# codeandkey/kami

Hardware: AMD Instinct MI355X
Metric: NN leaf-evals/sec at batch 512 (119×8×8 planes), 1/2/4/8 MI355X (higher is better)
Workload: dtype bf16

## Files before the change

### kami_amd/csrc/kh_internal.h

```cpp
#pragma once
#include <hip/hip_runtime.h>
#include <stddef.h>
#include <stdint.h>

#include "../../include/kami_hip.h"

namespace kh {

void launch_encode_f32(const kh_board* d_boards, int n, float* d_planes, hipStream_t s);

void launch_gather_legal(const float* policy, const int32_t* offsets, const int32_t* actions,
                         float* priors, int B, hipStream_t s, const float* vfull = nullptr, int vstride = 0,
                         float* values = nullptr, const int* flags_in = nullptr, int* flags_out = nullptr);

void launch_signal(unsigned* host_word, unsigned serial, hipStream_t s);

struct SimpleLayer {
    const float* wt;
    const float* scale;
    const float* shift;
    int Ci, Co, taps;
    int relu;
};
void launch_simple_conv(const SimpleLayer& L, const float* in, const float* skip, float* out,
                        int B, hipStream_t s);
void launch_softmax4672(const float* logits, float* policy, int B, int* flags, hipStream_t s);
void launch_value_fc(const float* v64, const float* fcw, const float* fcb, float* value_full,
                     int B, int* flags, hipStream_t s);

constexpr int TW_NB = 2;
constexpr int TW_CP = 64;

struct TowerArgs {
    const float* in;
    const kh_board* boards;
    int B, F, R;
    const char* wstream;
    int nchunks;
    const float* params;
    int npar;
    const float* fcw4;
    const float* fcb;
    float* policy;
    float* vfull;
    float* logits;
    int* flags;
// ... 60 lines not shown
```

### kami_amd/csrc/tower8_mfma.hip

```cpp
#include "tower_common.h"

#include <atomic>

namespace kh {

using f32x4_t = float __attribute__((ext_vector_type(4)));
__device__ __forceinline__ void store_wt(f32x4_t* p, f32x4_t v) { asm volatile("global_store_dwordx4 %0, %1, off sc1" ::"v"(p), "v"(v) : "memory"); }
__device__ __forceinline__ void store_wt(float* p, float v) { asm volatile("global_store_dword %0, %1, off sc1" ::"v"(p), "v"(v) : "memory"); }

constexpr int T8_LAG = 1;
struct CPipe { unsigned ring; int cslot; };

__device__ __forceinline__ unsigned cpipe_advance(CPipe& p)
{
    p.cslot = (p.cslot + 1 == RING_D) ? 0 : p.cslot + 1;
    return p.ring + p.cslot * CHUNK;
}

__device__ __forceinline__ unsigned cpipe_step(CPipe& p)
{
    asm volatile("s_barrier" ::: "memory");
    __builtin_amdgcn_sched_barrier(0);
    p.cslot = (p.cslot + 1 == RING_D) ? 0 : p.cslot + 1;
    return p.ring + p.cslot * CHUNK;
// ... 8 lines not shown
    asm volatile("s_mov_b32 %0, m0\n\ts_mov_b32 m0, %3\n\ts_nop 0\n\t"
                 "global_load_lds_dwordx4 %1, %2\n\tglobal_load_lds_dwordx4 %1, %2 offset:1024\n\t"
                 "global_load_lds_dwordx4 %1, %2 offset:2048\n\tglobal_load_lds_dwordx4 %1, %2 offset:3072\n\t"
                 "s_mov_b32 m0, %0"
                 : "=&s"(keep) : "v"(voff), "s"(sbase), "s"(dst) : "memory");
    p.next = (p.next + 1 == p.nch) ? 0 : p.next + 1;
    p.islot = (p.islot + 1 == RING_D) ? 0 : p.islot + 1;
}

template <int VMX>
__device__ __forceinline__ void hpipe_step(Pipe& p, int hw, int lane)
{
    asm volatile("s_waitcnt vmcnt(%0)" ::"n"(4 * (RING_D - 3 - T8_LAG) + VMX) : "memory");
    asm volatile("s_barrier" ::: "memory");
    pipe_issue4(p, hw, lane);
}

template <typename T, int TAPS, int KS, int MS, int PAR, int NREG = 0, bool CF = false, int TAILV = 0>
__device__ __forceinline__ void gemm8_layer(CPipe& p, const char* smem, int lane, unsigned b_base, int stride,
                                            f32x16 (&acc)[MS], typename Elem<T>::vec8 (&A)[2][8],
                                            const typename Elem<T>::vec8* breg = nullptr)
{
    using V = typename Elem<T>::vec8;
    using S = LayerShape<TAPS, KS, MS>;
    constexpr int KPC = S::KPC;
    constexpr int NF = KPC * MS;
    V B[2][KPC];
#pragma unroll
    for (int k = 0; k < KPC; ++k) {
        if (k < NREG) B[PAR][k] = breg[k];
        else B[PAR][k] = *reinterpret_cast<const V*>(smem + b_base + b_offset<TAPS, KS, CF>(k, stride));
    }
#pragma unroll
    for (int n = 0; n < S::NCH; ++n) {
        const int cur = (PAR + n) & 1, nxt = cur ^ 1;
        const unsigned a_off = cpipe_step(p) + lane * 16;
#pragma unroll
        for (int f = 0; f < 8; ++f)
            if (n + 1 == S::NCH || f < NF) A[nxt][f] = *reinterpret_cast<const V*>(smem + a_off + f * 1024);
        if (n + 1 < S::NCH) {
#pragma unroll
            for (int k = 0; k < KPC; ++k) {
                if ((n + 1) * KPC + k < NREG) B[nxt][k] = breg[(n + 1) * KPC + k];
                else B[nxt][k] = *reinterpret_cast<const V*>(smem + b_base + b_offset<TAPS, KS, CF>((n + 1) * KPC + k, stride));
            }
        }
        if (TAILV > 0 && n == S::NCH - 1) {
#pragma unroll
            for (int ms = 0; ms < MS; ++ms)
#pragma unroll
                for (int k = 0; k < KPC; ++k) acc[ms] = Elem<T>::mfma(A[cur][k * MS + ms], B[cur][k], acc[ms]);
#pragma unroll
            for (int i = 0; i < KPC; ++i) {
                __builtin_amdgcn_sched_group_barrier(0x100, 2, 0);
                __builtin_amdgcn_sched_group_barrier(0x008, 1, 0);
            }
#pragma unroll
            for (int i = 0; i < (MS - 1) * KPC; ++i) {
                __builtin_amdgcn_sched_group_barrier(0x008, 1, 0);
                if (i > 0) __builtin_amdgcn_sched_group_barrier(0x002, TAILV, 0);
            }
            continue;
        }
#pragma unroll
        for (int k = 0; k < KPC; ++k)
#pragma unroll
            for (int ms = 0; ms < MS; ++ms) acc[ms] = Elem<T>::mfma(A[cur][k * MS + ms], B[cur][k], acc[ms]);
#pragma unroll
        for (int i = 0; i < NF; ++i) {
            __builtin_amdgcn_sched_group_barrier(0x100, 2, 0);
            __builtin_amdgcn_sched_group_barrier(0x008, 1, 0);
        }
    }
}

template <typename T, int PAR>
__device__ __forceinline__ void gemm8_dummy(CPipe& p, const char* smem, int lane, typename Elem<T>::vec8 (&A)[2][8])
{
    using V = typename Elem<T>::vec8;
    const unsigned a_off = cpipe_step(p) + lane * 16;
#pragma unroll
    for (int f = 0; f < 8; ++f) A[PAR ^ 1][f] = *reinterpret_cast<const V*>(smem + a_off + f * 1024);
}


enum { BM_RASTER = 0, BM_CENTRE = 1, BM_QUARTERS = 2 };
template <int TAPS, int KS, int BM>
__device__ __forceinline__ constexpr unsigned b_off8(int kk, int stride)
// ... 166 lines not shown
    constexpr int cur = CURP, nxt = CURP ^ 1;
    const unsigned a_off = cpipe_step(p) + lane * 16;
    T8_RDA(nxt, 0, a_off); T8_RDA(nxt, 1, a_off); acc[0] = Elem<T>::mfma(A[cur][0], B[cur][0], acc[0]); T8_FENCE();
    T8_RDA(nxt, 2, a_off); T8_RDA(nxt, 3, a_off); acc[0] = Elem<T>::mfma(A[cur][2], B[cur][1], acc[0]); T8_FENCE();
    T8_RDA(nxt, 4, a_off); T8_RDA(nxt, 5, a_off); acc[0] = Elem<T>::mfma(A[cur][4], B[cur][2], acc[0]); T8_FENCE();
    T8_RDA(nxt, 6, a_off); T8_RDA(nxt, 7, a_off); acc[0] = Elem<T>::mfma(A[cur][6], B[cur][3], acc[0]); T8_FENCE();
    acc[1] = Elem<T>::mfma(A[cur][1], B[cur][0], acc[1]); T8_FENCE();
    acc[1] = Elem<T>::mfma(A[cur][3], B[cur][1], acc[1]); T8_FENCE();
    xk.o[0][0] = epi_group<T, EPI, 0>(acc[0], xf[0]); xk.o[0][1] = epi_group<T, EPI, 1>(acc[0], xf[0]);
    acc[1] = Elem<T>::mfma(A[cur][5], B[cur][2], acc[1]); T8_FENCE();
    xk.o[0][2] = epi_group<T, EPI, 2>(acc[0], xf[0]); xk.o[0][3] = epi_group<T, EPI, 3>(acc[0], xf[0]);
    acc[1] = Elem<T>::mfma(A[cur][7], B[cur][3], acc[1]); T8_FENCE();
    xk.o[1][0] = epi_group<T, EPI, 0>(acc[1], xf[1]); xk.o[1][1] = epi_group<T, EPI, 1>(acc[1], xf[1]);
    xk.o[1][2] = epi_group<T, EPI, 2>(acc[1], xf[1]); xk.o[1][3] = epi_group<T, EPI, 3>(acc[1], xf[1]);
}
#undef T8_RDA

template <int STRIDE>
__device__ __forceinline__ void zero_halo(char* base, int board_bytes, int t)
{
    const u32x4 z = { 0, 0, 0, 0 };
    for (int i = t; i < TW_NB * NPIX; i += 256) {
        const int pp = i % NPIX, yy = pp / PITCH, xx = pp % PITCH;
        if (yy >= 1 && yy <= 8 && xx >= 1 && xx <= 8) continue;
        char* d = base + (i / NPIX) * board_bytes + pp * STRIDE;
#pragma unroll
        for (int k = 0; k < STRIDE / 16; ++k) *reinterpret_cast<u32x4*>(d + k * 16) = z;
    }
}

// ... 41 lines not shown

template <typename T, int KS_STEM, bool LEGAL = false>
__global__ __launch_bounds__(512) void tower8_kernel(TowerArgs a)
{
    extern __shared__ __attribute__((aligned(16))) char smem[];
    constexpr int FP = KS_STEM * 16;
    constexpr int SSTR = FP * 2 + 16;
    constexpr int SBOARD = NPIX * SSTR;
    constexpr int ST_SIZE = st_size(FP);
    constexpr int LDS_PAR = LDS_ST + ST_SIZE;
    constexpr int LDS_L = LDS_X;
    using V = typename Elem<T>::vec8;
    constexpr int NSTEM = LayerShape<9, KS_STEM, 2>::NCH;
    constexpr int P1 = NSTEM & 1;
    constexpr int NLAYER = LayerShape<9, TW_CP / 16, 2>::NCH;
    constexpr int NPOL = LayerShape<1, TW_CP / 16, 4>::NCH + LayerShape<1, KH_POLICY_MID / 16, 3>::NCH + (P1 ? 1 : 0);

    const int tid = threadIdx.x;
    const int lane = tid & 63;
    const int wave = __builtin_amdgcn_readfirstlane(tid >> 6);
    const int ct = tid & 255;
    const int cw = wave & 3;
    const int R = a.R, F = a.F;

    float* par = reinterpret_cast<float*>(smem + LDS_PAR);
    const float* shift3 = par;
    const float* pshift1 = par + (1 + 2 * R) * TW_CP;
    const float* pbias2 = pshift1 + KH_POLICY_MID;
    const float* vw = pbias2 + 128;
    const float* vsh = vw + TW_CP;
    float* v64 = const_cast<float*>(vsh) + 4;
    float* red = v64 + TW_NB * 64;
    const int ngroups = (a.B + TW_NB - 1) / TW_NB;

    if (wave >= 6) {
        const int pt = tid & 127;
        for (int grp = blockIdx.x; grp < ngroups; grp += gridDim.x) {
            const int b0 = grp * TW_NB;
            if (KS_STEM == 8) {
                float4_u pl[4][8];
                const int lc = pt & 7;
                const int nb = min(TW_NB, a.B - b0);
                const char* gbase = reinterpret_cast<const char*>(a.in + (size_t)b0 * 64 * F);
                unsigned voff[8];
#pragma unroll
                for (int j = 0; j < 8; ++j) {
                    const int ip = (pt >> 3) + 16 * j;
                    voff[j] = (unsigned)((min(ip >> 6, nb - 1) * 64 + (ip & 63)) * F) * 4u;
                }
                const unsigned sdst = LDS_ST + ((((pt >> 6) + 1) * PITCH + ((pt >> 3) & 7) + 1) * SSTR) + 8 * lc;
                unsigned badmax = 0u;
// ... 92 lines not shown
                        for (int k = 0; k < 4; ++k) {
                            const float lo = vin[j][2 * k], hi = vin[j][2 * k + 1];
                            bad = bad || !__builtin_isfinite(lo) || !__builtin_isfinite(hi);
                            w[k] = pack2<T>(lo, hi);
                        }
                        o.x = w[0]; o.y = w[1]; o.z = w[2]; o.w = w[3];
                        *reinterpret_cast<u32x4*>(smem + LDS_ST + bb * SBOARD + (((p >> 3) + 1) * PITCH + (p & 7) + 1) * SSTR + (pt % CH) * 16) = o;
                    }
                    if (__any(bad) && lane == 0) raise_flag<LEGAL>(a, 0);
                }
                lds_barrier();
                for (int i = 0; i < NSTEM; ++i) asm volatile("s_barrier" ::: "memory");
            }
            const int nsteps = 2 * R * NLAYER + NPOL;
            for (int i = 0; i < nsteps; ++i) {
                asm volatile("s_barrier" ::: "memory");
                if (i == 0 && R > 0) {
                    for (int z = 0; z < 2; ++z) zero_halo<XSTR>(smem + LDS_ST, XBOARD, pt + 128 * z);
                    asm volatile("s_waitcnt lgkmcnt(0)" ::: "memory");
                }
            }
            helper_value_fc<LEGAL>(a, v64, b0, tid & 255, lane);
            asm volatile("s_barrier" ::: "memory");
        }
    } else if (wave >= 4) {
        const int hw = wave - 4;
        const int nsteps = NSTEM + 2 * R * NLAYER + NPOL;
        Pipe pipe;
        pipe.stream = a.wstream; pipe.nch = a.nchunks; pipe.next = 0; pipe.islot = 0; pipe.ring = LDS_RING;
#pragma unroll
        for (int i = 0; i < RING_D - 1; ++i) pipe_issue4(pipe, hw, lane);

        for (int grp = blockIdx.x; grp < ngroups; grp += gridDim.x) {
            asm volatile("s_waitcnt vmcnt(%0)\n\ts_barrier" ::"n"(4 * (RING_D - 3)) : "memory");
            for (int i = 0; i < nsteps; ++i) hpipe_step<0>(pipe, hw, lane);
// ... 55 lines not shown
                constexpr int BMS = KS_STEM == 8 ? BM_QUARTERS : BM_RASTER;
#pragma unroll
                for (int k = 0; k < 4; ++k) B[0][k] = *reinterpret_cast<const V*>(smem + sin + b_off8<9, KS_STEM, BMS>(k, SSTR));
                gemm8_steps<T, 9, KS_STEM, 2, 0, 0, BMS, 0, NSTEM - 1>(pipe, smem, lane, sin, SSTR, accA, A, B);
            }
            constexpr int CP1 = P1 ^ 1;
            for (int r = 0; r < R; ++r) {
                boundary<T, EPI_RESID, CP1>(pipe, smem, lane, accA, accB, sh0 + (1 + 2 * r) * TW_CP * 4, A, B, xf, xout_h, xin);
                gemm8_steps<T, 9, TW_CP / 16, 2, P1, 4, BM_CENTRE, 1, 8, true>(pipe, smem, lane, xin, XSTR, accB, A, B);
                boundary<T, EPI_PACK, P1>(pipe, smem, lane, accB, accA, sh0 + (2 + 2 * r) * TW_CP * 4, A, B, xf, tout_h, tin);
                gemm8_steps<T, 9, TW_CP / 16, 2, P1 ^ 1, 4, BM_CENTRE, 1, 8, true>(pipe, smem, lane, tin, XSTR, accA, A, B);
            }
            tower_tail<T, EPI_RESID, CP1>(pipe, smem, lane, accA, A, B, xf, xk);

            {
                f32x2 s01 = { 0.0f, 0.0f }, s23 = { 0.0f, 0.0f };
#pragma unroll
                for (int ms = 0; ms < 2; ++ms)
#pragma unroll
                    for (int g = 0; g < 4; ++g) {
                        using f32x4 = float __attribute__((ext_vector_type(4)));
                        const f32x4 w = *reinterpret_cast<const f32x4*>(vw + ms * 32 + 8 * g + 4 * h);
                        const f32x2 x01 = { xf[ms][4 * g + 0], xf[ms][4 * g + 1] }, x23 = { xf[ms][4 * g + 2], xf[ms][4 * g + 3] };
                        s01 = x01 * w.xy + s01;
                        s23 = x23 * w.zw + s23;
                    }
                const float part = (s01.x + s01.y) + (s23.x + s23.y);
                const unsigned pu = __float_as_uint(part);
                if ((pu & 0x7f800000u) == 0x7f800000u) raise_flag<LEGAL>(a, 0);
                const auto sw = __builtin_amdgcn_permlane32_swap(pu, pu, false, false);
                const float sv = __uint_as_float(sw[0]) + __uint_as_float(sw[1]);
                if (h == 0) v64[wb * 64 + py * 8 + px] = relu_nan(sv + vsh[0]);
            }

            Packed<4> pk;
            {
                f32x16 acc[4];
                V bf[4];
                packed_fragments<T, 2>(xk, bf);
                acc_init<4>(acc, pshift1, h);
                asm volatile("s_waitcnt lgkmcnt(0)" ::: "memory");
                gemm8_layer<T, 1, TW_CP / 16, 4, P1, 4>(pipe, smem, lane, 0, 0, acc, A, bf);
                epilogue_pack<T, 4>(acc, pk);
            }
            {
                f32x16 acc[3];
                V bf[8];
                packed_fragments<T, 4>(pk, bf);
                acc_init<3>(acc, pbias2, h);
                gemm8_layer<T, 1, KH_POLICY_MID / 16, 3, P1, 8>(pipe, smem, lane, 0, 0, acc, A, bf);
                if (P1) gemm8_dummy<T, 1>(pipe, smem, lane, A);
                float* lrow = reinterpret_cast<float*>(smem + LDS_L + wb * LBOARD) + (py * 8 + px) * KH_POLICY_PLANES;
                float m = -INFINITY;
#pragma unroll
                for (int ms = 0; ms < 3; ++ms)
#pragma unroll
                    for (int g = 0; g < 4; ++g)
#pragma unroll
                        for (int i = 0; i < 4; ++i) {
                            const int plane = ms * 32 + 8 * g + 4 * h + i;
                            if (plane < KH_POLICY_PLANES) {
                                lrow[plane] = acc[ms][4 * g + i];
                                m = fmaxf(m, acc[ms][4 * g + i]);
                            }
                        }
                m = wave_max_f(m);
                if (lane == 0) red[cw] = m;
                lds_barrier();
            }

            {
                const int bb = ct >> 7, tt = ct & 127;
                const bool live = (b0 + bb) < a.B;
                const float4* L4 = reinterpret_cast<const float4*>(smem + LDS_L + bb * LBOARD);
                constexpr int NQ = KH_PSIZE / 4;
                float4 v[10];
#pragma unroll
                for (int k = 0; k < 10; ++k) {
                    const int q = tt + 128 * k;
                    v[k] = (q < NQ) ? L4[q] : make_float4(-INFINITY, -INFINITY, -INFINITY, -INFINITY);
// ... 86 lines not shown
```

### kami_amd/csrc/weights.hip

```cpp
#include "engine.h"
#include "blob_layout.h"
#include "weights_pack.h"

#include <algorithm>
#include <atomic>
#include <cmath>
#include <cstring>
#include <thread>

namespace kh {
namespace {

struct ConvBN { const float *w, *b, *g, *be, *rm, *rv; };
struct HostNet {
    ConvBN stem;
    std::vector<ConvBN> res;
    ConvBN pconv;
    const float *p2w, *p2b;
    ConvBN vconv;
    const float *fcw, *fcb;
};

HostNet parse_blob(const float* blob, int F, int C, int R)
{
// ... 12 lines not shown
    n.fcw = take();
    n.fcb = take();
    return n;
}

void fold_bn(const ConvBN& c, int co, float* scale, float* shift)
{
    for (int i = 0; i < co; ++i) {
        const float s = c.g[i] / sqrtf(c.rv[i] + 1e-5f);
        scale[i] = s;
        shift[i] = (c.b[i] - c.rm[i]) * s + c.be[i];
    }
}

void pack_layer(std::vector<uint16_t>& out, int dtype, const float* w, const float* scale, int Co, int Ci,
                int taps, int KS, int MS, int ci0 = 0, bool centre_first = false, int perm = 0)
{
    int kstep = 0;
    for (int ti = 0; ti < taps; ++ti) {
        const int tap = !centre_first ? ti : (ti == 0 ? 4 : (ti <= 4 ? ti - 1 : ti));
        for (int ks = 0; ks < KS; ++ks, ++kstep)
            for (int ms = 0; ms < MS; ++ms)
                for (int l = 0; l < 64; ++l) {
                    const int r = l & 31, h = l >> 5;
                    for (int j = 0; j < 8; ++j) {
                        const int co = ms * 32 + r;
                        const int ci = ci0 + (kstep < perm ? 32 * (ks >> 1) + 8 * (2 * (ks & 1) + (j >> 2)) + 4 * h + (j & 3)
                                                           : ks * 16 + 8 * h + j);
                        float v = 0.0f;
                        if (co < Co && ci < Ci) v = w[((size_t)co * Ci + ci) * taps + tap] * (scale ? scale[co] : 1.0f);
                        out.push_back(dtype == KH_BF16 ? f2bf16(v) : f2f16(v));
                    }
                }
    }
}

void pack_layer_generic(uint16_t* o, int dtype, const float* w, const float* scale,
                        int Co, int Ci, int taps, int CoP, int CiP)
{
    const bool bf = dtype == KH_BF16;
    for (int cb = 0; cb < CoP / 64; ++cb)
        for (int slice = 0; slice < CiP / 64; ++slice)
            for (int tap = 0; tap < taps; ++tap)
                for (int kk = 0; kk < 4; ++kk)
                    for (int ms = 0; ms < 2; ++ms)
                        for (int l = 0; l < 64; ++l) {
                            const int r = l & 31, h = l >> 5, ks = slice * 4 + kk;
                            const int co = cb * 64 + ms * 32 + r, ci0 = ks * 16 + 8 * h;
// ... 45 lines not shown

enum Buf { B_TW_STREAM, B_TW_PAR, B_TW_FC4, B_LY_W, B_LY_W4, B_LY_W2B, B_LY_WH, B_LY_SHIFT, B_LY_MISC, B_SIMPLE, NBUF };

DevMem& buf_of(Weights& W, int b)
{
    DevMem* m[NBUF] = { &W.tw_stream, &W.tw_par, &W.tw_fc4, &W.ly_w, &W.ly_w4, &W.ly_w2b, &W.ly_wh, &W.ly_shift, &W.ly_misc, &W.simple };
    return *m[b];
}

struct FoldItem { ConvBN c; int co; };
struct FoldRef { int item = -1, shift = 0; };
struct PackItem {
    int buf; size_t off, bytes;
    int kind; const float* w; int fold;
    int Co, Ci, taps;
    int KS, MS, ci0, centre_first, perm, chunk_frags;
    int CoP, CiP, CBC;
};
struct CopyItem {
    int buf; size_t off;
    int kind; const float* src; FoldRef fsrc;
    int scale_of;
    int n, npad, Co, Ci, taps;
};
struct SimpleOff { size_t wt, scale, shift; int Ci, Co, taps, relu; };
struct Plan {
    int dtype = KH_F32, fold_stride = 0;
    std::vector<FoldItem> folds;
    std::vector<PackItem> packs;
    std::vector<CopyItem> copies;
    size_t bytes[NBUF] = {};
// ... 29 lines not shown
void copy_fc4(Plan& P, int buf, size_t off, const float* fcw)
{
    copy_item(P, buf, off, CP_FC4, fcw, {}, KH_VALUE_WIDTH * 64, KH_VALUE_WIDTH * 64);
}

int plan_layers(Plan& P, Weights& W, const HostNet& n, int dtype, int F, int C, int R)
{
    const bool f32 = dtype == KH_F32;
    const int FP = f32 ? (F + 7) / 8 * 8 : (F + 63) / 64 * 64, CP = (C + 63) / 64 * 64;
    if (CP > 256 || FP > 256) return KH_OK;
    const size_t el = f32 ? 4 : 2;
    size_t nw = 0, nw4 = 0, nwh = 0, nw2b = 0, nshift = 0;
    const bool want2b = !f32 && CP == 256 && FP == 128;
    auto blocks = [&](int buf, size_t& at, int kind, const float* wt, int fold, int Co, int Ci, int taps, int CoP, int CiP, int CBC) {
        const size_t nel = (size_t)CoP * CiP * taps;
        P.packs.push_back({ buf, at * el, nel * el, kind, wt, fold, Co, Ci, taps, 0, 0, 0, 0, 0, 8, CoP, CiP, CBC });
        at += nel;
        P.bytes[buf] = at * el;
    };
    auto add = [&](const float* wt, int fold, int Co, int Ci, int taps, int CoP, int CiP) {
        W.ly_shift_off.push_back(nshift);
        W.ly_w4_off.push_back((size_t)-1);
        W.ly_w_off.push_back(nw);
        if (f32) blocks(B_LY_W, nw, PK_F32, wt, fold, Co, Ci, taps, CoP, CiP, 64);
        else {
            blocks(B_LY_W, nw, PK_BLOCKS, wt, fold, Co, Ci, taps, CoP, CiP, 64);
            if (taps == 9 && CoP % 128 == 0 && (CiP == 128 || CiP == 256)) {
                W.ly_w4_off.back() = nw4;
                blocks(B_LY_W4, nw4, PK_BLOCKS, wt, fold, Co, Ci, taps, CoP, CiP, 128);
            }
            if (want2b && taps == 9) blocks(B_LY_W2B, nw2b, PK_BLOCKS, wt, fold, Co, Ci, taps, CoP, CiP, 256);
// ... 22 lines not shown
    W.ly_FP = FP; W.ly_CP = CP;
    W.ly_ok = true;
    P.threads = true;
    return KH_OK;
}

int plan_tower(Plan& P, Weights& W, const HostNet& n, int F, int C, int R)
{
    if (C > TW_CP) { W.tw_why = "filters > 64 not supported by the MFMA tower kernel yet"; return KH_OK; }
    if (F > 128) { W.tw_why = "features > 128 not supported by the MFMA tower kernel yet"; return KH_OK; }
    const int FP = F <= 32 ? 32 : 128;
    if (tower_lds_bytes(FP, R) > 160 * 1024) { W.tw_why = "too many residual blocks for the LDS parameter area"; return KH_OK; }
    constexpr size_t FRAG = 512;
    size_t at = 0;
    auto stream = [&](const float* w, int fold, int Co, int Ci, int taps, int KS, int MS, int ci0, bool centre_first, int perm,
                      int chunk_frags, bool pad) {
        const size_t frags = (size_t)taps * KS * MS;
        const size_t out = chunk_frags < 8 ? frags / chunk_frags * 8 : (pad ? (frags + 7) / 8 * 8 : frags);
        P.packs.push_back({ B_TW_STREAM, at * 2, out * FRAG * 2, PK_STREAM, w, fold, Co, Ci, taps, KS, MS, ci0, centre_first, perm, chunk_frags, 0, 0, 0 });
        at += out * FRAG;
    };
    if (FP == 128) {
        for (int q = 0; q < 4; ++q) stream(n.stem.w, P.f_stem(), C, F, 9, 2, 2, 32 * q, false, 0, 8, false);
        if (at != (size_t)18 * 4096) return fail(KH_ERR_INVALID, "internal: stem stream size");
    } else {
        stream(n.stem.w, P.f_stem(), C, F, 9, FP / 16, 2, 0, false, 0, 8, true);
    }
    for (int i = 0; i < 2 * R; ++i) stream(n.res[i].w, P.f_res(i), C, C, 9, TW_CP / 16, 2, 0, true, TW_CP / 16, 8, true);
    stream(n.pconv.w, P.f_pconv(), KH_POLICY_MID, C, 1, TW_CP / 16, 4, 0, false, TW_CP / 16, 8, true);
    static_assert((KH_POLICY_MID / 16 * 3) % 6 == 0, "policyconv2 fills whole chunks of 6 fragments");
    stream(n.p2w, -1, KH_POLICY_PLANES, KH_POLICY_MID, 1, KH_POLICY_MID / 16, 3, 0, false, KH_POLICY_MID / 16, 6, false);
    if (at % 4096) return fail(KH_ERR_INVALID, "internal: weight stream is not whole chunks");
    if (((at / 4096) & 1) != 0) stream(nullptr, -1, 0, 0, 1, 1, 8, 0, false, 0, 8, true);
    P.bytes[B_TW_STREAM] = at * 2;

    size_t p = 0;
    copy_item(P, B_TW_PAR, p, CP_COPY, nullptr, { P.f_stem(), 1 }, C, TW_CP);
    p += TW_CP;
    for (int i = 0; i < 2 * R; ++i, p += TW_CP) copy_item(P, B_TW_PAR, p, CP_COPY, nullptr, { P.f_res(i), 1 }, C, TW_CP);
    copy_item(P, B_TW_PAR, p, CP_COPY, nullptr, { P.f_pconv(), 1 }, KH_POLICY_MID, 128);
    p += 128;
    copy_item(P, B_TW_PAR, p, CP_COPY, n.p2b, {}, KH_POLICY_PLANES, 128);
    p += 128;
    copy_item(P, B_TW_PAR, p, CP_MULS, n.vconv.w, {}, C, TW_CP, P.f_vconv());
    p += TW_CP;
    copy_item(P, B_TW_PAR, p, CP_COPY, nullptr, { P.f_vconv(), 1 }, 1, 4);
// ... 70 lines not shown
    else for (int i = 0; i < f.co; ++i) { scale[i] = 1.0f; shift[i] = f.c.b[i]; }
}

void pack_host(const Plan& P, const PackItem& it, const float* fold, char* dst)
{
    const float* sc = it.fold < 0 ? nullptr : fold + P.fold_at({ it.fold, 0 });
    if (it.kind == PK_F32) return pack_layer_f32(reinterpret_cast<float*>(dst), it.w, sc, it.Co, it.Ci, it.taps, it.CoP, it.CiP);
    uint16_t* o = reinterpret_cast<uint16_t*>(dst);
    if (it.kind == PK_BLOCKS) {
        if (it.CBC == 64) pack_layer_generic(o, P.dtype, it.w, sc, it.Co, it.Ci, it.taps, it.CoP, it.CiP);
        else pack_layer_wide128(o, P.dtype, it.w, sc, it.Co, it.Ci, it.taps, it.CoP, it.CiP, it.CBC);
        return;
    }
    constexpr size_t FRAG = 512;
    std::vector<uint16_t> f;
    pack_layer(f, P.dtype, it.w, sc, it.Co, it.Ci, it.taps, it.KS, it.MS, it.ci0, it.centre_first != 0, it.perm);
    if (it.chunk_frags == 8) { memcpy(o, f.data(), f.size() * 2); return; }
    for (size_t c = 0; c * it.chunk_frags * FRAG < f.size(); ++c)
        memcpy(o + c * 8 * FRAG, f.data() + c * it.chunk_frags * FRAG, it.chunk_frags * FRAG * 2);
}

void copy_host(const Plan& P, const CopyItem& it, const float* fold, float* dst)
{
    const float* src = it.fsrc.item < 0 ? it.src : fold + P.fold_at(it.fsrc);
    if (it.kind == CP_COPY) memcpy(dst, src, sizeof(float) * it.n);
    else if (it.kind == CP_MULS) {
        const float s = fold[P.fold_at({ it.scale_of, 0 })];
        for (int i = 0; i < it.n; ++i) dst[i] = src[i] * s;
    } else if (it.kind == CP_FC4) {
        for (int j = 0; j < KH_VALUE_WIDTH; ++j)
            for (int k = 0; k < 64; ++k) dst[((size_t)(k / 4) * KH_VALUE_WIDTH + j) * 4 + (k & 3)] = src[(size_t)j * 64 + k];
// ... 46 lines not shown
    CopyJob* cj = reinterpret_cast<CopyJob*>(tables.data() + at_c);
    for (size_t i = 0; i < nf; ++i) {
        const ConvBN& c = P.folds[i].c;
        fj[i] = { c.b, c.g, c.be, c.rm, c.rv, d_fold + P.fold_at({ (int)i, 0 }), d_fold + P.fold_at({ (int)i, 1 }), P.folds[i].co };
    }
    unsigned pblocks = 0, cblocks = 0;
    for (size_t i = 0; i < np; ++i) {
        const PackItem& it = P.packs[i];
        PackJob& j = pj[i];
        j.w = it.w;
        j.scale = it.fold < 0 ? nullptr : d_fold + P.fold_at({ it.fold, 0 });
        j.dst = buf_of(W, it.buf).as<char>() + it.off;
        j.groups = (unsigned)(it.bytes / 16);
        j.block0 = pblocks;
        j.kind = it.kind; j.dtype = P.dtype; j.Co = it.Co; j.Ci = it.Ci; j.taps = it.taps;
        j.KS = it.KS; j.MS = it.MS; j.ci0 = it.ci0; j.centre_first = it.centre_first; j.perm = it.perm; j.chunk_frags = it.chunk_frags;
        j.CiP = it.CiP; j.CBC = it.CBC;
        pblocks += (j.groups + PACK_THREADS - 1) / PACK_THREADS;
    }
    for (size_t i = 0; i < nc; ++i) {
        const CopyItem& it = P.copies[i];
        CopyJob& j = cj[i];
        j.src = it.fsrc.item < 0 ? it.src : d_fold + P.fold_at(it.fsrc);
        j.s = it.scale_of < 0 ? nullptr : d_fold + P.fold_at({ it.scale_of, 0 });
        j.dst = buf_of(W, it.buf).as<float>() + it.off;
        j.n = (unsigned)it.n; j.npad = (unsigned)it.npad;
        j.block0 = cblocks;
        j.kind = it.kind; j.Co = it.Co; j.Ci = it.Ci; j.taps = it.taps;
        cblocks += (j.npad + PACK_THREADS - 1) / PACK_THREADS;
    }
    HIPCHK(hipMemcpyAsync(d_tab, tables.data(), tables.size(), hipMemcpyHostToDevice, st));
// ... 99 lines not shown
```

### kami_amd/csrc/weights_pack.h

```cpp
#pragma once
#include "kh_internal.h"

namespace kh {

__host__ __device__ inline uint16_t f2bf16(float f)
{
    uint32_t u;
    __builtin_memcpy(&u, &f, 4);
    if ((u & 0x7fffffffu) > 0x7f800000u) return (uint16_t)((u >> 16) | 0x40);
    u += 0x7fffu + ((u >> 16) & 1u);
    return (uint16_t)(u >> 16);
}
__host__ __device__ inline uint16_t f2f16(float f)
{
    _Float16 h = (_Float16)f;
    uint16_t r;
    __builtin_memcpy(&r, &h, 2);
    return r;
}

struct FoldJob {
    const float *b, *g, *be, *rm, *rv;
    float *scale, *shift;
    int co;
};

enum { PK_STREAM = 0, PK_BLOCKS = 1, PK_F32 = 2 };
struct PackJob {
    const float* w;
    const float* scale;
    void* dst;
    unsigned groups;
    unsigned block0;
    int kind, dtype, Co, Ci, taps;
    int KS, MS, ci0, centre_first, perm, chunk_frags;
    int CiP, CBC;
};

enum { CP_COPY = 0, CP_MULS = 1, CP_FC4 = 2, CP_TRANSPOSE = 3 };
struct CopyJob {
    const float* src;
    const float* s;
    float* dst;
    unsigned n, npad;
    unsigned block0;
    int kind, Co, Ci, taps;
};

constexpr int PACK_THREADS = 256;

// ... 6 lines not shown
```

### kami_amd/csrc/weights_pack.hip

```cpp
#include "weights_pack.h"

namespace kh {
namespace {

__global__ void __launch_bounds__(PACK_THREADS) fold_kernel(const FoldJob* __restrict__ jobs)
{
    const FoldJob jb = jobs[blockIdx.x];
    for (int i = threadIdx.x; i < jb.co; i += PACK_THREADS) {
        if (!jb.g) { jb.scale[i] = 1.0f; jb.shift[i] = jb.b[i]; continue; }
        const float s = jb.g[i] / sqrtf(jb.rv[i] + 1e-5f);
        const float d = jb.b[i] - jb.rm[i];
        const float p = d * s;
        jb.scale[i] = s;
        jb.shift[i] = p + jb.be[i];
    }
}

template <class J> __device__ inline int find_job(const J* jobs, int njobs, unsigned block)
{
    int lo = 0, hi = njobs - 1;
    while (lo < hi) {
        const int mid = (lo + hi + 1) >> 1;
        if (jobs[mid].block0 <= block) lo = mid; else hi = mid - 1;
    }
// ... 25 lines not shown
        const int co = cb * 64 + ms * 32 + r;
        float4 v;
        v.x = element(jb, co, j * 8 + 4 * h + 0, tap);
        v.y = element(jb, co, j * 8 + 4 * h + 1, tap);
        v.z = element(jb, co, j * 8 + 4 * h + 2, tap);
        v.w = element(jb, co, j * 8 + 4 * h + 3, tap);
        static_cast<float4*>(jb.dst)[g] = v;
        return;
    }
    int co = 0, tap = 0, ks = 0;
    bool live = true, permuted = false;
    if (jb.kind == PK_STREAM) {
        const unsigned frag = g >> 6, chunk = frag >> 3, fi = frag & 7;
        const unsigned sf = chunk * jb.chunk_frags + fi;
        live = (int)fi < jb.chunk_frags && sf < (unsigned)(jb.taps * jb.KS * jb.MS);
        const int ti = sf / (jb.KS * jb.MS), ms = sf % jb.MS;
        ks = (sf / jb.MS) % jb.KS;
        tap = !jb.centre_first ? ti : (ti == 0 ? 4 : (ti <= 4 ? ti - 1 : ti));
        permuted = ti * jb.KS + ks < jb.perm;
        co = ms * 32 + r;
    } else {
        const int M = jb.CBC / 32, slices = jb.CiP / 64;
        unsigned t = g >> 6;
        const int ms = t % M; t /= M;
        const int kk = t & 3; t >>= 2;
        tap = t % jb.taps; t /= jb.taps;
        const int slice = t % slices, cb = t / slices;
        ks = slice * 4 + kk;
        co = cb * jb.CBC + ms * 32 + r;
    }
    uint16_t o[8];
#pragma unroll
// ... 54 lines not shown
```

Before: 15.64 million.

## Fuse and hand-schedule policy heads with tile-major weight streams and distributed halo zeroing

Replaces the generic gemm8_layer calls for the two policy convolutions and the value-head reduction with a hand-interleaved policy_heads routine. It overlaps LDS fragment reads, bias init, value dot-products, packing and logit stores with MFMA issue. The policy weight streams are repacked tile-major into whole 8-fragment chunks, which changes the pipeline chunk count. Helper waves now zero the halo one slice per barrier step instead of all at once on the first step. This adds a lot of fragile hand scheduling and layout coupling between the packer and the kernel.

```diff
diff --git a/kami_amd/csrc/kh_internal.h b/kami_amd/csrc/kh_internal.h
--- a/kami_amd/csrc/kh_internal.h
+++ b/kami_amd/csrc/kh_internal.h
@@ -30,6 +30,8 @@
 
 constexpr int TW_NB = 2;
 constexpr int TW_CP = 64;
+constexpr int POLICY1_CHUNKS = 4 * (TW_CP / 16) / 8;
+constexpr int POLICY2_CHUNKS = 3 * (KH_POLICY_MID / 16) / 8;
 
 struct TowerArgs {
     const float* in;
diff --git a/kami_amd/csrc/tower8_mfma.hip b/kami_amd/csrc/tower8_mfma.hip
--- a/kami_amd/csrc/tower8_mfma.hip
+++ b/kami_amd/csrc/tower8_mfma.hip
@@ -46,64 +46,6 @@
     asm volatile("s_waitcnt vmcnt(%0)" ::"n"(4 * (RING_D - 3 - T8_LAG) + VMX) : "memory");
     asm volatile("s_barrier" ::: "memory");
     pipe_issue4(p, hw, lane);
-}
-
-template <typename T, int TAPS, int KS, int MS, int PAR, int NREG = 0, bool CF = false, int TAILV = 0>
-__device__ __forceinline__ void gemm8_layer(CPipe& p, const char* smem, int lane, unsigned b_base, int stride,
-                                            f32x16 (&acc)[MS], typename Elem<T>::vec8 (&A)[2][8],
-                                            const typename Elem<T>::vec8* breg = nullptr)
-{
-    using V = typename Elem<T>::vec8;
-    using S = LayerShape<TAPS, KS, MS>;
-    constexpr int KPC = S::KPC;
-    constexpr int NF = KPC * MS;
-    V B[2][KPC];
-#pragma unroll
-    for (int k = 0; k < KPC; ++k) {
-        if (k < NREG) B[PAR][k] = breg[k];
-        else B[PAR][k] = *reinterpret_cast<const V*>(smem + b_base + b_offset<TAPS, KS, CF>(k, stride));
-    }
-#pragma unroll
-    for (int n = 0; n < S::NCH; ++n) {
-        const int cur = (PAR + n) & 1, nxt = cur ^ 1;
-        const unsigned a_off = cpipe_step(p) + lane * 16;
-#pragma unroll
-        for (int f = 0; f < 8; ++f)
-            if (n + 1 == S::NCH || f < NF) A[nxt][f] = *reinterpret_cast<const V*>(smem + a_off + f * 1024);
-        if (n + 1 < S::NCH) {
-#pragma unroll
-            for (int k = 0; k < KPC; ++k) {
-                if ((n + 1) * KPC + k < NREG) B[nxt][k] = breg[(n + 1) * KPC + k];
-                else B[nxt][k] = *reinterpret_cast<const V*>(smem + b_base + b_offset<TAPS, KS, CF>((n + 1) * KPC + k, stride));
-            }
-        }
-        if (TAILV > 0 && n == S::NCH - 1) {
-#pragma unroll
-            for (int ms = 0; ms < MS; ++ms)
-#pragma unroll
-                for (int k = 0; k < KPC; ++k) acc[ms] = Elem<T>::mfma(A[cur][k * MS + ms], B[cur][k], acc[ms]);
-#pragma unroll
-            for (int i = 0; i < KPC; ++i) {
-                __builtin_amdgcn_sched_group_barrier(0x100, 2, 0);
-                __builtin_amdgcn_sched_group_barrier(0x008, 1, 0);
-            }
-#pragma unroll
-            for (int i = 0; i < (MS - 1) * KPC; ++i) {
-                __builtin_amdgcn_sched_group_barrier(0x008, 1, 0);
-                if (i > 0) __builtin_amdgcn_sched_group_barrier(0x002, TAILV, 0);
-            }
-            continue;
-        }
-#pragma unroll
-        for (int k = 0; k < KPC; ++k)
-#pragma unroll
-            for (int ms = 0; ms < MS; ++ms) acc[ms] = Elem<T>::mfma(A[cur][k * MS + ms], B[cur][k], acc[ms]);
-#pragma unroll
-        for (int i = 0; i < NF; ++i) {
-            __builtin_amdgcn_sched_group_barrier(0x100, 2, 0);
-            __builtin_amdgcn_sched_group_barrier(0x008, 1, 0);
-        }
-    }
 }
 
 template <typename T, int PAR>
@@ -300,6 +242,120 @@
     xk.o[1][0] = epi_group<T, EPI, 0>(acc[1], xf[1]); xk.o[1][1] = epi_group<T, EPI, 1>(acc[1], xf[1]);
     xk.o[1][2] = epi_group<T, EPI, 2>(acc[1], xf[1]); xk.o[1][3] = epi_group<T, EPI, 3>(acc[1], xf[1]);
 }
+
+template <typename T, int PAR, bool LEGAL>
+__device__ __forceinline__ float policy_heads(CPipe& p, char* smem, int lane, int h, const TowerArgs& a, typename Elem<T>::vec8 (&A)[2][8],
+                                              const Packed<2>& xk, const f32x16 (&xf)[2], unsigned hb, const float* vsh, float* vdst, float* lrow)
+{
+    using V = typename Elem<T>::vec8;
+    using f32x4 = float __attribute__((ext_vector_type(4)));
+    constexpr int c0 = PAR, c1 = PAR ^ 1;
+    constexpr int O_BIAS2 = KH_POLICY_MID * 4, O_VW = O_BIAS2 + 128 * 4;
+#define T8_LD4(acc, g, off) do { const float4 s_ = *reinterpret_cast<const float4*>(smem + hb + (off)); \
+        acc[4 * (g) + 0] = s_.x; acc[4 * (g) + 1] = s_.y; acc[4 * (g) + 2] = s_.z; acc[4 * (g) + 3] = s_.w; } while (0)
+#define T8_INIT(acc, ms, g, base) T8_LD4(acc, g, (base) + ((ms) * 32 + 8 * (g)) * 4)
+#define T8_LDV(ms, g) (vwr[ms][g] = *reinterpret_cast<const f32x4*>(smem + hb + O_VW + ((ms) * 32 + 8 * (g)) * 4))
+#define T8_PACK(ms, g) do { pk.o[ms][g].x = relu_pk(pack2<T>(acc[ms][4 * (g) + 0], acc[ms][4 * (g) + 1])); \
+                            pk.o[ms][g].y = relu_pk(pack2<T>(acc[ms][4 * (g) + 2], acc[ms][4 * (g) + 3])); \
+                            T8_PIN(pk.o[ms][g].x); T8_PIN(pk.o[ms][g].y); } while (0)
+#define T8_PFRAG(ks) __builtin_bit_cast(V, (u32x4){ pk.o[(ks) >> 1][2 * ((ks) & 1)].x, pk.o[(ks) >> 1][2 * ((ks) & 1)].y, \
+                                                    pk.o[(ks) >> 1][2 * ((ks) & 1) + 1].x, pk.o[(ks) >> 1][2 * ((ks) & 1) + 1].y })
+#define T8_LOGITS(q, ms, g) do { _Pragma("unroll") for (int i_ = 0; i_ < 4; ++i_) { \
+            const int plane_ = (ms) * 32 + 8 * (g) + i_;       \
+            if ((ms) < 2 || plane_ + 4 * h < KH_POLICY_PLANES) { lrow[plane_] = q[4 * (g) + i_]; m = fmaxf(m, q[4 * (g) + i_]); } } T8_PIN(m); } while (0)
+#define T8_PIN(x) asm volatile("" : "+v"(x))
+#define T8_MF(acc, a, b) do { acc = Elem<T>::mfma(a, b, acc); T8_PIN(acc); T8_FENCE(); } while (0)
+    f32x16 acc[4];
+    Packed<4> pk;
+    V bf[4];
+    f32x4 vwr[2][4];
+    packed_fragments<T, 2>(xk, bf);
+    lrow += 4 * h;
+#pragma unroll
+    for (int g = 0; g < 4; ++g) T8_INIT(acc[0], 0, g, 0);
+
+    unsigned a_off = cpipe_step(p) + lane * 16;
+    f32x2 s01 = { 0.0f, 0.0f }, s23 = { 0.0f, 0.0f };
+#define T8_VFMA(ms, g) do { const f32x2 x01_ = { xf[ms][4 * (g) + 0], xf[ms][4 * (g) + 1] }, x23_ = { xf[ms][4 * (g) + 2], xf[ms][4 * (g) + 3] }; \
+        s01 = x01_ * vwr[ms][g].xy + s01; s23 = x23_ * vwr[ms][g].zw + s23; T8_PIN(s01); T8_PIN(s23); } while (0)
+    T8_RDA(c1, 0, a_off); T8_RDA(c1, 1, a_off); T8_INIT(acc[1], 1, 0, 0); T8_INIT(acc[1], 1, 1, 0); T8_MF(acc[0], A[c0][0], bf[0]);
+    T8_RDA(c1, 2, a_off); T8_RDA(c1, 3, a_off); T8_INIT(acc[1], 1, 2, 0); T8_INIT(acc[1], 1, 3, 0); T8_MF(acc[0], A[c0][1], bf[1]);
+    T8_RDA(c1, 4, a_off); T8_RDA(c1, 5, a_off); T8_LDV(0, 0); T8_LDV(0, 1); T8_MF(acc[0], A[c0][2], bf[2]);
+    T8_RDA(c1, 6, a_off); T8_RDA(c1, 7, a_off); T8_LDV(0, 2); T8_LDV(0, 3); T8_MF(acc[0], A[c0][3], bf[3]);
+    T8_LDV(1, 0); T8_LDV(1, 1); T8_LDV(1, 2); T8_LDV(1, 3);
+    T8_VFMA(0, 0); T8_VFMA(0, 1); T8_VFMA(0, 2); T8_VFMA(0, 3); T8_MF(acc[1], A[c0][4], bf[0]);
+    T8_VFMA(1, 0); T8_VFMA(1, 1); T8_VFMA(1, 2); T8_VFMA(1, 3); T8_MF(acc[1], A[c0][5], bf[1]);
+    const float part = (s01.x + s01.y) + (s23.x + s23.y);
+    const unsigned pu = __float_as_uint(part);
+    const float vshift = vsh[0];
+#pragma unroll
+    for (int g = 0; g < 4; ++g) T8_INIT(acc[2], 2, g, 0);
+    T8_MF(acc[1], A[c0][6], bf[2]);
+    if ((pu & 0x7f800000u) == 0x7f800000u) raise_flag<LEGAL>(a, 0);
+    T8_FENCE();
+    {
+        const auto sw = __builtin_amdgcn_permlane32_swap(pu, pu, false, false);
+        const float sv = __uint_as_float(sw[0]) + __uint_as_float(sw[1]);
+        *vdst = relu_nan(sv + vshift);
+    }
+#pragma unroll
+    for (int g = 0; g < 4; ++g) T8_INIT(acc[3], 3, g, 0);
+    T8_MF(acc[1], A[c0][7], bf[3]);
+#undef T8_VFMA
+
+    f32x16 q0, q1, q2;
+    float m = -INFINITY;
+    a_off = cpipe_step(p) + lane * 16;
+    T8_RDA(c0, 0, a_off); T8_RDA(c0, 1, a_off); T8_PACK(0, 0); T8_PACK(0, 1); T8_MF(acc[2], A[c1][0], bf[0]);
+    T8_RDA(c0, 2, a_off); T8_RDA(c0, 3, a_off); T8_PACK(0, 2); T8_PACK(0, 3); T8_MF(acc[2], A[c1][1], bf[1]);
+    T8_RDA(c0, 4, a_off); T8_RDA(c0, 5, a_off); T8_PACK(1, 0); T8_PACK(1, 1); T8_MF(acc[2], A[c1][2], bf[2]);
+    T8_RDA(c0, 6, a_off); T8_RDA(c0, 7, a_off); T8_PACK(1, 2); T8_PACK(1, 3); T8_MF(acc[2], A[c1][3], bf[3]);
+    T8_INIT(q0, 0, 0, O_BIAS2); T8_INIT(q0, 0, 1, O_BIAS2); T8_MF(acc[3], A[c1][4], bf[0]);
+    T8_INIT(q0, 0, 2, O_BIAS2); T8_INIT(q0, 0, 3, O_BIAS2); T8_MF(acc[3], A[c1][5], bf[1]);
+    T8_PACK(2, 0); T8_PACK(2, 1); T8_MF(acc[3], A[c1][6], bf[2]);
+    T8_PACK(2, 2); T8_PACK(2, 3); T8_MF(acc[3], A[c1][7], bf[3]);
+
+    a_off = cpipe_step(p) + lane * 16;
+    T8_RDA(c1, 0, a_off); T8_RDA(c1, 1, a_off); T8_MF(q0, A[c0][0], T8_PFRAG(0));
+    T8_RDA(c1, 2, a_off); T8_RDA(c1, 3, a_off); T8_PACK(3, 0); T8_PACK(3, 1); T8_MF(q0, A[c0][1], T8_PFRAG(1));
+    T8_RDA(c1, 4, a_off); T8_RDA(c1, 5, a_off); T8_PACK(3, 2); T8_PACK(3, 3); T8_MF(q0, A[c0][2], T8_PFRAG(2));
+    T8_RDA(c1, 6, a_off); T8_RDA(c1, 7, a_off); T8_MF(q0, A[c0][3], T8_PFRAG(3));
+    T8_INIT(q1, 1, 0, O_BIAS2); T8_INIT(q1, 1, 1, O_BIAS2); T8_MF(q0, A[c0][4], T8_PFRAG(4));
+    T8_INIT(q1, 1, 2, O_BIAS2); T8_INIT(q1, 1, 3, O_BIAS2); T8_MF(q0, A[c0][5], T8_PFRAG(5));
+    T8_MF(q0, A[c0][6], T8_PFRAG(6));
+    T8_MF(q0, A[c0][7], T8_PFRAG(7));
+
+    a_off = cpipe_step(p) + lane * 16;
+    T8_RDA(c0, 0, a_off); T8_RDA(c0, 1, a_off); T8_INIT(q2, 2, 0, O_BIAS2); T8_INIT(q2, 2, 1, O_BIAS2); T8_MF(q1, A[c1][0], T8_PFRAG(0));
+    T8_RDA(c0, 2, a_off); T8_RDA(c0, 3, a_off); T8_INIT(q2, 2, 2, O_BIAS2); T8_INIT(q2, 2, 3, O_BIAS2); T8_MF(q1, A[c1][1], T8_PFRAG(1));
+    T8_RDA(c0, 4, a_off); T8_RDA(c0, 5, a_off); T8_MF(q1, A[c1][2], T8_PFRAG(2));
+    T8_RDA(c0, 6, a_off); T8_RDA(c0, 7, a_off); T8_MF(q1, A[c1][3], T8_PFRAG(3));
+    T8_LOGITS(q0, 0, 0); T8_MF(q1, A[c1][4], T8_PFRAG(4));
+    T8_LOGITS(q0, 0, 1); T8_MF(q1, A[c1][5], T8_PFRAG(5));
+    T8_LOGITS(q0, 0, 2); T8_MF(q1, A[c1][6], T8_PFRAG(6));
+    T8_LOGITS(q0, 0, 3); T8_MF(q1, A[c1][7], T8_PFRAG(7));
+
+    a_off = cpipe_step(p) + lane * 16;
+    T8_RDA(c1, 0, a_off); T8_RDA(c1, 1, a_off); T8_MF(q2, A[c0][0], T8_PFRAG(0));
+    T8_RDA(c1, 2, a_off); T8_RDA(c1, 3, a_off); T8_MF(q2, A[c0][1], T8_PFRAG(1));
+    T8_RDA(c1, 4, a_off); T8_RDA(c1, 5, a_off); T8_MF(q2, A[c0][2], T8_PFRAG(2));
+    T8_RDA(c1, 6, a_off); T8_RDA(c1, 7, a_off); T8_MF(q2, A[c0][3], T8_PFRAG(3));
+    T8_LOGITS(q1, 1, 0); T8_MF(q2, A[c0][4], T8_PFRAG(4));
+    T8_LOGITS(q1, 1, 1); T8_MF(q2, A[c0][5], T8_PFRAG(5));
+    T8_LOGITS(q1, 1, 2); T8_MF(q2, A[c0][6], T8_PFRAG(6));
+    T8_LOGITS(q1, 1, 3); T8_MF(q2, A[c0][7], T8_PFRAG(7));
+    if (c1 == 1) gemm8_dummy<T, 1>(p, smem, lane, A);
+    T8_LOGITS(q2, 2, 0); T8_LOGITS(q2, 2, 1);
+    return m;
+#undef T8_PIN
+#undef T8_MF
+#undef T8_LD4
+#undef T8_INIT
+#undef T8_LDV
+#undef T8_PACK
+#undef T8_PFRAG
+#undef T8_LOGITS
+}
 #undef T8_RDA
 
 template <int STRIDE>
@@ -371,7 +427,9 @@
     constexpr int NSTEM = LayerShape<9, KS_STEM, 2>::NCH;
     constexpr int P1 = NSTEM & 1;
     constexpr int NLAYER = LayerShape<9, TW_CP / 16, 2>::NCH;
-    constexpr int NPOL = LayerShape<1, TW_CP / 16, 4>::NCH + LayerShape<1, KH_POLICY_MID / 16, 3>::NCH + (P1 ? 1 : 0);
+    constexpr bool PARITY_CHUNK = ((NSTEM + POLICY1_CHUNKS + POLICY2_CHUNKS) & 1) != 0;
+    constexpr int NPOL = POLICY1_CHUNKS + POLICY2_CHUNKS + (PARITY_CHUNK ? 1 : 0);
+    static_assert(POLICY1_CHUNKS == 2 && POLICY2_CHUNKS == 3 && PARITY_CHUNK == (P1 == 0), "policy_heads walks two + three chunks");
 
     const int tid = threadIdx.x;
     const int lane = tid & 63;
@@ -392,6 +450,15 @@
 
     if (wave >= 6) {
         const int pt = tid & 127;
+        constexpr int T_HALO_STEPS = TW_CP * 2 / 16;
+        static_assert(T_HALO_STEPS < NLAYER, "T's halo is complete within conv1 of the first block");
+        unsigned t_halo = 0;
+        if (R > 0 && pt < TW_NB * (NPIX - 64)) {
+            const int bb = pt / (NPIX - 64), q = pt % (NPIX - 64);
+            const int pp = q < PITCH ? q : q >= PITCH + 32 ? 9 * PITCH + (q - PITCH - 32)
+                                         : (((q - PITCH) >> 2) + 1) * PITCH + (((q - PITCH) & 3) ? 8 + ((q - PITCH) & 3) : 0);
+            t_halo = LDS_ST + bb * XBOARD + pp * XSTR;
+        }
         for (int grp = blockIdx.x; grp < ngroups; grp += gridDim.x) {
             const int b0 = grp * TW_NB;
             if (KS_STEM == 8) {
@@ -514,11 +581,9 @@
             }
             const int nsteps = 2 * R * NLAYER + NPOL;
             for (int i = 0; i < nsteps; ++i) {
+                if (i == T_HALO_STEPS) asm volatile("s_waitcnt lgkmcnt(0)" ::: "memory");
                 asm volatile("s_barrier" ::: "memory");
-                if (i == 0 && R > 0) {
-                    for (int z = 0; z < 2; ++z) zero_halo<XSTR>(smem + LDS_ST, XBOARD, pt + 128 * z);
-                    asm volatile("s_waitcnt lgkmcnt(0)" ::: "memory");
-                }
+                if (i < T_HALO_STEPS && t_halo) *reinterpret_cast<u32x4*>(smem + t_halo + 16 * i) = (u32x4){ 0, 0, 0, 0 };
             }
             helper_value_fc<LEGAL>(a, v64, b0, tid & 255, lane);
             asm volatile("s_barrier" ::: "memory");
@@ -604,56 +669,9 @@
             tower_tail<T, EPI_RESID, CP1>(pipe, smem, lane, accA, A, B, xf, xk);
 
             {
-                f32x2 s01 = { 0.0f, 0.0f }, s23 = { 0.0f, 0.0f };
-#pragma unroll
-                for (int ms = 0; ms < 2; ++ms)
-#pragma unroll
-                    for (int g = 0; g < 4; ++g) {
-                        using f32x4 = float __attribute__((ext_vector_type(4)));
-                        const f32x4 w = *reinterpret_cast<const f32x4*>(vw + ms * 32 + 8 * g + 4 * h);
-                        const f32x2 x01 = { xf[ms][4 * g + 0], xf[ms][4 * g + 1] }, x23 = { xf[ms][4 * g + 2], xf[ms][4 * g + 3] };
-                        s01 = x01 * w.xy + s01;
-                        s23 = x23 * w.zw + s23;
-                    }
-                const float part = (s01.x + s01.y) + (s23.x + s23.y);
-                const unsigned pu = __float_as_uint(part);
-                if ((pu & 0x7f800000u) == 0x7f800000u) raise_flag<LEGAL>(a, 0);
-                const auto sw = __builtin_amdgcn_permlane32_swap(pu, pu, false, false);
-                const float sv = __uint_as_float(sw[0]) + __uint_as_float(sw[1]);
-                if (h == 0) v64[wb * 64 + py * 8 + px] = relu_nan(sv + vsh[0]);
-            }
-
-            Packed<4> pk;
-            {
-                f32x16 acc[4];
-                V bf[4];
-                packed_fragments<T, 2>(xk, bf);
-                acc_init<4>(acc, pshift1, h);
-                asm volatile("s_waitcnt lgkmcnt(0)" ::: "memory");
-                gemm8_layer<T, 1, TW_CP / 16, 4, P1, 4>(pipe, smem, lane, 0, 0, acc, A, bf);
-                epilogue_pack<T, 4>(acc, pk);
-            }
-            {
-                f32x16 acc[3];
-                V bf[8];
-                packed_fragments<T, 4>(pk, bf);
-                acc_init<3>(acc, pbias2, h);
-                gemm8_layer<T, 1, KH_POLICY_MID / 16, 3, P1, 8>(pipe, smem, lane, 0, 0, acc, A, bf);
-                if (P1) gemm8_dummy<T, 1>(pipe, smem, lane, A);
                 float* lrow = reinterpret_cast<float*>(smem + LDS_L + wb * LBOARD) + (py * 8 + px) * KH_POLICY_PLANES;
-                float m = -INFINITY;
-#pragma unroll
-                for (int ms = 0; ms < 3; ++ms)
-#pragma unroll
-                    for (int g = 0; g < 4; ++g)
-#pragma unroll
-                        for (int i = 0; i < 4; ++i) {
-                            const int plane = ms * 32 + 8 * g + 4 * h + i;
-                            if (plane < KH_POLICY_PLANES) {
-                                lrow[plane] = acc[ms][4 * g + i];
-                                m = fmaxf(m, acc[ms][4 * g + i]);
-                            }
-                        }
+                float m = policy_heads<T, P1, LEGAL>(pipe, smem, lane, h, a, A, xk, xf, sh0 + (1 + 2 * R) * TW_CP * 4, vsh,
+                                                     v64 + wb * 64 + py * 8 + px, lrow);
                 m = wave_max_f(m);
                 if (lane == 0) red[cw] = m;
                 lds_barrier();
diff --git a/kami_amd/csrc/weights.hip b/kami_amd/csrc/weights.hip
--- a/kami_amd/csrc/weights.hip
+++ b/kami_amd/csrc/weights.hip
@@ -50,24 +50,24 @@
 }
 
 void pack_layer(std::vector<uint16_t>& out, int dtype, const float* w, const float* scale, int Co, int Ci,
-                int taps, int KS, int MS, int ci0 = 0, bool centre_first = false, int perm = 0)
-{
-    int kstep = 0;
+                int taps, int KS, int MS, int ci0 = 0, bool centre_first = false, int perm = 0, bool tile_major = false)
+{
     for (int ti = 0; ti < taps; ++ti) {
         const int tap = !centre_first ? ti : (ti == 0 ? 4 : (ti <= 4 ? ti - 1 : ti));
-        for (int ks = 0; ks < KS; ++ks, ++kstep)
-            for (int ms = 0; ms < MS; ++ms)
-                for (int l = 0; l < 64; ++l) {
-                    const int r = l & 31, h = l >> 5;
-                    for (int j = 0; j < 8; ++j) {
-                        const int co = ms * 32 + r;
-                        const int ci = ci0 + (kstep < perm ? 32 * (ks >> 1) + 8 * (2 * (ks & 1) + (j >> 2)) + 4 * h + (j & 3)
-                                                           : ks * 16 + 8 * h + j);
-                        float v = 0.0f;
-                        if (co < Co && ci < Ci) v = w[((size_t)co * Ci + ci) * taps + tap] * (scale ? scale[co] : 1.0f);
-                        out.push_back(dtype == KH_BF16 ? f2bf16(v) : f2f16(v));
-                    }
+        for (int f = 0; f < KS * MS; ++f) {
+            const int ks = tile_major ? f % KS : f / MS, ms = tile_major ? f / KS : f % MS, kstep = ti * KS + ks;
+            for (int l = 0; l < 64; ++l) {
+                const int r = l & 31, h = l >> 5;
+                for (int j = 0; j < 8; ++j) {
+                    const int co = ms * 32 + r;
+                    const int ci = ci0 + (kstep < perm ? 32 * (ks >> 1) + 8 * (2 * (ks & 1) + (j >> 2)) + 4 * h + (j & 3)
+                                                       : ks * 16 + 8 * h + j);
+                    float v = 0.0f;
+                    if (co < Co && ci < Ci) v = w[((size_t)co * Ci + ci) * taps + tap] * (scale ? scale[co] : 1.0f);
+                    out.push_back(dtype == KH_BF16 ? f2bf16(v) : f2f16(v));
                 }
+            }
+        }
     }
 }
 
@@ -143,7 +143,7 @@
     int buf; size_t off, bytes;
     int kind; const float* w; int fold;
     int Co, Ci, taps;
-    int KS, MS, ci0, centre_first, perm, chunk_frags;
+    int KS, MS, ci0, centre_first, perm, chunk_frags, tile_major;
     int CoP, CiP, CBC;
 };
 struct CopyItem {
@@ -203,7 +203,7 @@
     const bool want2b = !f32 && CP == 256 && FP == 128;
     auto blocks = [&](int buf, size_t& at, int kind, const float* wt, int fold, int Co, int Ci, int taps, int CoP, int CiP, int CBC) {
         const size_t nel = (size_t)CoP * CiP * taps;
-        P.packs.push_back({ buf, at * el, nel * el, kind, wt, fold, Co, Ci, taps, 0, 0, 0, 0, 0, 8, CoP, CiP, CBC });
+        P.packs.push_back({ buf, at * el, nel * el, kind, wt, fold, Co, Ci, taps, 0, 0, 0, 0, 0, 8, 0, CoP, CiP, CBC });
         at += nel;
         P.bytes[buf] = at * el;
     };
@@ -256,10 +256,10 @@
     constexpr size_t FRAG = 512;
     size_t at = 0;
     auto stream = [&](const float* w, int fold, int Co, int Ci, int taps, int KS, int MS, int ci0, bool centre_first, int perm,
-                      int chunk_frags, bool pad) {
+                      int chunk_frags, bool pad, bool tile_major = false) {
         const size_t frags = (size_t)taps * KS * MS;
         const size_t out = chunk_frags < 8 ? frags / chunk_frags * 8 : (pad ? (frags + 7) / 8 * 8 : frags);
-        P.packs.push_back({ B_TW_STREAM, at * 2, out * FRAG * 2, PK_STREAM, w, fold, Co, Ci, taps, KS, MS, ci0, centre_first, perm, chunk_frags, 0, 0, 0 });
+        P.packs.push_back({ B_TW_STREAM, at * 2, out * FRAG * 2, PK_STREAM, w, fold, Co, Ci, taps, KS, MS, ci0, centre_first, perm, chunk_frags, tile_major, 0, 0, 0 });
         at += out * FRAG;
     };
     if (FP == 128) {
@@ -269,9 +269,9 @@
         stream(n.stem.w, P.f_stem(), C, F, 9, FP / 16, 2, 0, false, 0, 8, true);
     }
     for (int i = 0; i < 2 * R; ++i) stream(n.res[i].w, P.f_res(i), C, C, 9, TW_CP / 16, 2, 0, true, TW_CP / 16, 8, true);
-    stream(n.pconv.w, P.f_pconv(), KH_POLICY_MID, C, 1, TW_CP / 16, 4, 0, false, TW_CP / 16, 8, true);
-    static_assert((KH_POLICY_MID / 16 * 3) % 6 == 0, "policyconv2 fills whole chunks of 6 fragments");
-    stream(n.p2w, -1, KH_POLICY_PLANES, KH_POLICY_MID, 1, KH_POLICY_MID / 16, 3, 0, false, KH_POLICY_MID / 16, 6, false);
+    static_assert(POLICY1_CHUNKS * 8 == TW_CP / 16 * 4 && POLICY2_CHUNKS * 8 == KH_POLICY_MID / 16 * 3, "policy streams fill whole chunks");
+    stream(n.pconv.w, P.f_pconv(), KH_POLICY_MID, C, 1, TW_CP / 16, 4, 0, false, TW_CP / 16, 8, false, true);
+    stream(n.p2w, -1, KH_POLICY_PLANES, KH_POLICY_MID, 1, KH_POLICY_MID / 16, 3, 0, false, KH_POLICY_MID / 16, 8, false, true);
     if (at % 4096) return fail(KH_ERR_INVALID, "internal: weight stream is not whole chunks");
     if (((at / 4096) & 1) != 0) stream(nullptr, -1, 0, 0, 1, 1, 8, 0, false, 0, 8, true);
     P.bytes[B_TW_STREAM] = at * 2;
@@ -372,7 +372,7 @@
     }
     constexpr size_t FRAG = 512;
     std::vector<uint16_t> f;
-    pack_layer(f, P.dtype, it.w, sc, it.Co, it.Ci, it.taps, it.KS, it.MS, it.ci0, it.centre_first != 0, it.perm);
+    pack_layer(f, P.dtype, it.w, sc, it.Co, it.Ci, it.taps, it.KS, it.MS, it.ci0, it.centre_first != 0, it.perm, it.tile_major != 0);
     if (it.chunk_frags == 8) { memcpy(o, f.data(), f.size() * 2); return; }
     for (size_t c = 0; c * it.chunk_frags * FRAG < f.size(); ++c)
         memcpy(o + c * 8 * FRAG, f.data() + c * it.chunk_frags * FRAG, it.chunk_frags * FRAG * 2);
@@ -449,7 +449,7 @@
         j.groups = (unsigned)(it.bytes / 16);
         j.block0 = pblocks;
         j.kind = it.kind; j.dtype = P.dtype; j.Co = it.Co; j.Ci = it.Ci; j.taps = it.taps;
-        j.KS = it.KS; j.MS = it.MS; j.ci0 = it.ci0; j.centre_first = it.centre_first; j.perm = it.perm; j.chunk_frags = it.chunk_frags;
+        j.KS = it.KS; j.MS = it.MS; j.ci0 = it.ci0; j.centre_first = it.centre_first; j.perm = it.perm; j.chunk_frags = it.chunk_frags; j.tile_major = it.tile_major;
         j.CiP = it.CiP; j.CBC = it.CBC;
         pblocks += (j.groups + PACK_THREADS - 1) / PACK_THREADS;
     }
diff --git a/kami_amd/csrc/weights_pack.h b/kami_amd/csrc/weights_pack.h
--- a/kami_amd/csrc/weights_pack.h
+++ b/kami_amd/csrc/weights_pack.h
@@ -33,7 +33,7 @@
     unsigned groups;
     unsigned block0;
     int kind, dtype, Co, Ci, taps;
-    int KS, MS, ci0, centre_first, perm, chunk_frags;
+    int KS, MS, ci0, centre_first, perm, chunk_frags, tile_major;
     int CiP, CBC;
 };
 
diff --git a/kami_amd/csrc/weights_pack.hip b/kami_amd/csrc/weights_pack.hip
--- a/kami_amd/csrc/weights_pack.hip
+++ b/kami_amd/csrc/weights_pack.hip
@@ -63,8 +63,9 @@
         const unsigned frag = g >> 6, chunk = frag >> 3, fi = frag & 7;
         const unsigned sf = chunk * jb.chunk_frags + fi;
         live = (int)fi < jb.chunk_frags && sf < (unsigned)(jb.taps * jb.KS * jb.MS);
-        const int ti = sf / (jb.KS * jb.MS), ms = sf % jb.MS;
-        ks = (sf / jb.MS) % jb.KS;
+        const int ti = sf / (jb.KS * jb.MS), f = sf % (jb.KS * jb.MS);
+        const int ms = jb.tile_major ? f / jb.KS : f % jb.MS;
+        ks = jb.tile_major ? f % jb.KS : f / jb.MS;
         tap = !jb.centre_first ? ti : (ti == 0 ? 4 : (ti <= 4 ? ti - 1 : ti));
         permuted = ti * jb.KS + ks < jb.perm;
         co = ms * 32 + r;
```

Result: no change. 15.60 million (-0.2%).
